# Wells-Group/pmg-dolfinx

Hardware: AMD Instinct MI355X
Metric: DoFs/sec per p-MG V-cycle (Poisson, hex, p=4) (higher is better)
Workload: dtype f64; 1 GPU; Poisson p=4 V-cycle p=4->2->1, Chebyshev(3)/Jacobi, 64^3 hexes per GPU; fine_dofs_global=16974593, partition=1x1x1 bricks, 1 ghost-cell layer, exchange=none (single rank), rccl_ranks=1, comm_ranks=1

## Files before the change

include/pmg_amd.h:

```cpp
#ifndef PMG_AMD_H
#define PMG_AMD_H

#include <stddef.h>
#include <stdint.h>

#ifdef __cplusplus
extern "C" {
#endif

#define PMG_OK 0
#define PMG_ERR_INVALID -1
#define PMG_ERR_HIP -2
#define PMG_ERR_NUMERIC -3
#define PMG_MAX_DEGREE 8

typedef void* pmg_stream;

typedef struct pmg_layout_s* pmg_layout;
typedef struct pmg_comm_s* pmg_comm;
typedef struct pmg_laplacian_s* pmg_laplacian;
typedef struct pmg_chebyshev_s* pmg_chebyshev;
typedef struct pmg_cg_s* pmg_cg;
typedef struct pmg_interpolator_s* pmg_interpolator;
typedef struct pmg_multigrid_s* pmg_multigrid;
// ... 177 lines not shown
                                          const int32_t* bcells, int32_t n_bcells,
                                          pmg_laplacian fine_operator, pmg_stream stream);
int pmg_interpolator_create_ordered(pmg_interpolator* out, pmg_layout layout_coarse, pmg_layout layout_fine,
                                    int degree_coarse, int degree_fine, int32_t ncells,
                                    const int32_t* dofmap_coarse, const int32_t* dofmap_fine,
                                    const int32_t* lcells, int32_t n_lcells, const int32_t* bcells,
                                    int32_t n_bcells, pmg_laplacian fine_operator, int node_order,
                                    const int32_t* custom_coarse, const int32_t* custom_fine, pmg_stream stream);
int pmg_interpolator_destroy(pmg_interpolator ip);
int pmg_interpolator_interpolate(pmg_interpolator ip, double* coarse, double* fine,
                                 pmg_stream stream);
int pmg_interpolator_interpolate_add(pmg_interpolator ip, double* coarse, double* fine,
                                     pmg_stream stream);
int pmg_interpolator_reverse_interpolate(pmg_interpolator ip, double* fine, double* coarse,
                                         pmg_stream stream);
int pmg_interpolator_interpolate_add_f32(pmg_interpolator ip, const float* coarse, float* fine, pmg_stream stream);
int pmg_interpolator_reverse_interpolate_f32(pmg_interpolator ip, const float* fine, const float* fine_sub,
                                             float* coarse, pmg_stream stream);

int pmg_multigrid_create(pmg_multigrid* out, int nlevels, const pmg_layout* layouts,
                         const int8_t* bc_marker_coarsest);
int pmg_multigrid_destroy(pmg_multigrid mg);
int pmg_multigrid_set_operators(pmg_multigrid mg, const pmg_laplacian* ops);
int pmg_multigrid_set_solvers(pmg_multigrid mg, const pmg_chebyshev* smoothers);
int pmg_multigrid_set_interpolators(pmg_multigrid mg, const pmg_interpolator* interp);
int pmg_multigrid_set_coarse_solver(pmg_multigrid mg, pmg_cg coarse);
typedef int (*pmg_coarse_solve_fn)(void* user, double* x, double* b, pmg_stream stream);
int pmg_multigrid_set_coarse_callback(pmg_multigrid mg, pmg_coarse_solve_fn solve, void* user);
int pmg_amg_create(pmg_amg* out, pmg_laplacian op, pmg_stream stream);
int pmg_amg_create_replicated(pmg_amg* out, pmg_laplacian op, const int64_t* global_index, int64_t n_global,
// ... 6 lines not shown
int pmg_amg_set_krylov(pmg_amg amg, int max_iter, double rtol);
int pmg_amg_set_distributed_fine_level(pmg_amg amg, int enable);
int pmg_amg_solve(pmg_amg amg, double* x, const double* b, int* iterations, pmg_stream stream);
int pmg_amg_cycle(pmg_amg amg, double* x, const double* b, pmg_stream stream);
int pmg_amg_num_levels(pmg_amg amg);
int pmg_amg_level_info(pmg_amg amg, int level, long long* rows, long long* nnz, double* lambda_max);
int pmg_amg_export(pmg_amg amg, int level, int which, long long* rows, long long* cols, long long* nnz,
                   int32_t* rowptr, int32_t* colidx, double* values);
int pmg_multigrid_set_coarse_amg(pmg_multigrid mg, pmg_amg amg);

int pmg_multigrid_apply(pmg_multigrid mg, const double* rhs, double* y, double* rnorm,
                        pmg_stream stream);
int pmg_multigrid_set_graph(pmg_multigrid mg, int enable);
long long pmg_multigrid_graph_replays(pmg_multigrid mg);
int pmg_multigrid_apply_counts(pmg_multigrid mg, int* counts, int capacity);
#define PMG_PRECISION_FP64 0
#define PMG_PRECISION_FP32 1
int pmg_multigrid_set_precision(pmg_multigrid mg, int precision);
int pmg_multigrid_set_level_matrix(pmg_multigrid mg, int level, pmg_matrix M);
int pmg_multigrid_precision(pmg_multigrid mg);

#ifdef __cplusplus
}
#endif
#endif
```

pmg-dolfinx_amd/_lib.py:

```python
from __future__ import annotations

import ctypes as C
import os

_HERE = os.path.dirname(os.path.abspath(__file__))
LIB_PATH = os.environ.get("PMG_AMD_LIB") or os.path.join(_HERE, "lib", "libpmg_amd.so")

c_dp = C.POINTER(C.c_double)
c_ip = C.POINTER(C.c_int32)
c_bp = C.POINTER(C.c_int8)
c_lp = C.POINTER(C.c_int64)
vp = C.c_void_p

EXCHANGE_FN = C.CFUNCTYPE(C.c_int, vp, C.c_int, vp)
ALLREDUCE_FN = C.CFUNCTYPE(C.c_int, vp, c_dp, C.c_int)
COARSE_FN = C.CFUNCTYPE(C.c_int, vp, vp, vp, vp)


class PmgError(RuntimeError):
    """A pmg_* call returned non-zero; the message is ``pmg_last_error()``."""


_SIGS = {
    "pmg_last_error": (C.c_char_p, []),
# ... 107 lines not shown
        [C.POINTER(vp), vp, vp, C.c_int, C.c_int, C.c_int32, vp, vp, c_ip, C.c_int32, c_ip, C.c_int32, vp],
    ),
    "pmg_interpolator_create_with_operator": (
        C.c_int,
        [C.POINTER(vp), vp, vp, C.c_int, C.c_int, C.c_int32, vp, vp, c_ip, C.c_int32, c_ip, C.c_int32, vp, vp],
    ),
    "pmg_interpolator_create_ordered": (
        C.c_int,
        [C.POINTER(vp), vp, vp, C.c_int, C.c_int, C.c_int32, vp, vp, c_ip, C.c_int32, c_ip, C.c_int32, vp, C.c_int,
         c_ip, c_ip, vp],
    ),
    "pmg_interpolator_interpolate_add": (C.c_int, [vp, vp, vp, vp]),
    "pmg_interpolator_destroy": (C.c_int, [vp]),
    "pmg_interpolator_interpolate": (C.c_int, [vp, vp, vp, vp]),
    "pmg_interpolator_reverse_interpolate": (C.c_int, [vp, vp, vp, vp]),
    "pmg_interpolator_interpolate_add_f32": (C.c_int, [vp, vp, vp, vp]),
    "pmg_interpolator_reverse_interpolate_f32": (C.c_int, [vp, vp, vp, vp, vp]),
    "pmg_multigrid_create": (C.c_int, [C.POINTER(vp), C.c_int, C.POINTER(vp), vp]),
    "pmg_multigrid_destroy": (C.c_int, [vp]),
    "pmg_multigrid_set_operators": (C.c_int, [vp, C.POINTER(vp)]),
    "pmg_multigrid_set_solvers": (C.c_int, [vp, C.POINTER(vp)]),
    "pmg_multigrid_set_interpolators": (C.c_int, [vp, C.POINTER(vp)]),
    "pmg_multigrid_set_coarse_solver": (C.c_int, [vp, vp]),
    "pmg_multigrid_set_coarse_callback": (C.c_int, [vp, COARSE_FN, vp]),
    "pmg_multigrid_set_coarse_amg": (C.c_int, [vp, vp]),
    "pmg_multigrid_set_precision": (C.c_int, [vp, C.c_int]),
    "pmg_multigrid_precision": (C.c_int, [vp]),
    "pmg_amg_create": (C.c_int, [C.POINTER(vp), vp, vp]),
    "pmg_amg_create_replicated": (C.c_int, [C.POINTER(vp), vp, C.POINTER(C.c_int64), C.c_int64, vp]),
    "pmg_amg_create_distributed": (C.c_int, [C.POINTER(vp), vp, C.POINTER(C.c_int64), C.c_int64, vp]),
# ... 2 lines not shown
    "pmg_amg_set_cycles": (C.c_int, [vp, C.c_int]),
    "pmg_amg_set_krylov": (C.c_int, [vp, C.c_int, C.c_double]),
    "pmg_amg_set_distributed_fine_level": (C.c_int, [vp, C.c_int]),
    "pmg_amg_solve": (C.c_int, [vp, vp, vp, C.POINTER(C.c_int), vp]),
    "pmg_amg_cycle": (C.c_int, [vp, vp, vp, vp]),
    "pmg_amg_num_levels": (C.c_int, [vp]),
    "pmg_amg_level_info": (C.c_int, [vp, C.c_int, C.POINTER(C.c_longlong), C.POINTER(C.c_longlong), c_dp]),
    "pmg_amg_export": (C.c_int, [vp, C.c_int, C.c_int, C.POINTER(C.c_longlong), C.POINTER(C.c_longlong),
                                 C.POINTER(C.c_longlong), c_ip, c_ip, c_dp]),
    "pmg_laplacian_set_geometry_batch": (C.c_int, [vp, C.c_longlong]),
    "pmg_laplacian_geometry_bytes": (C.c_longlong, [vp]),
    "pmg_multigrid_apply": (C.c_int, [vp, vp, vp, c_dp, vp]),
    "pmg_multigrid_apply_counts": (C.c_int, [vp, C.POINTER(C.c_int), C.c_int]),
    "pmg_multigrid_set_graph": (C.c_int, [vp, C.c_int]),
    "pmg_multigrid_graph_replays": (C.c_longlong, [vp]),
    "pmg_matrix_create_from_laplacian": (C.c_int, [C.POINTER(vp), vp, vp]),
    "pmg_matrix_destroy": (C.c_int, [vp]),
    "pmg_matrix_update_values": (C.c_int, [vp, vp]),
    "pmg_matrix_apply": (C.c_int, [vp, vp, vp, vp]),
    "pmg_matrix_get_diag_inverse": (C.c_int, [vp, vp, vp]),
    "pmg_matrix_rows": (C.c_longlong, [vp]),
    "pmg_matrix_nnz": (C.c_longlong, [vp]),
    "pmg_matrix_bytes": (C.c_longlong, [vp]),
    "pmg_matrix_frobenius_norm": (C.c_int, [vp, c_dp]),
    "pmg_matrix_export": (C.c_int, [vp, C.POINTER(C.c_longlong), C.POINTER(C.c_longlong), c_ip, c_ip, c_dp]),
    "pmg_chebyshev_solve_matrix": (C.c_int, [vp, vp, vp, vp, vp]),
    "pmg_cg_solve_matrix": (C.c_int, [vp, vp, vp, vp, vp, C.POINTER(C.c_int), vp]),
    "pmg_multigrid_set_level_matrix": (C.c_int, [vp, C.c_int, vp]),
}

_COUNT_FUNCS = {"pmg_multigrid_graph_replays", "pmg_amg_num_levels", "pmg_laplacian_geometry_bytes", "pmg_comm_rank", "pmg_comm_size", "pmg_comm_capture_overlaps", "pmg_cg_coefficients", "pmg_cg_compute_eigenvalues", "pmg_multigrid_apply_counts", "pmg_version",
                "pmg_laplacian_degree", "pmg_multigrid_precision", "pmg_laplacian_launches_per_apply", "pmg_laplacian_apply_streams", "pmg_laplacian_is_affine",
                "pmg_laplacian_has_coefficient_field", "pmg_laplacian_lift_cell_count",
                "pmg_laplacian_chain_available", "pmg_laplacian_chain_form",
                "pmg_laplacian_node_order", "pmg_layout_forward_scatters",
                "pmg_matrix_rows", "pmg_matrix_nnz", "pmg_matrix_bytes"}

_lib = None


def exported_symbols():
    return sorted(_SIGS)


def lib():
    global _lib
    if _lib is None:
        if not os.path.exists(LIB_PATH):
            raise RuntimeError(
                f"{LIB_PATH} is missing: the HIP library has not been built. "
                "Run `python -c 'import __graft_entry__ as g; g.build()'` at the repo root. "
# ... 44 lines not shown
```

pmg-dolfinx_amd/csrc/common.hpp:

```cpp
#pragma once

#include "../../include/pmg_amd.h"

#include <hip/hip_runtime.h>

#include <cstdarg>
#include <cstdio>
#include <functional>
#include <string>
#include <vector>

namespace pmg
{
extern thread_local std::string g_last_error;

int fail(int code, const char* fmt, ...);

#define PMG_HIP(call)                                                                              \
  do                                                                                               \
  {                                                                                                \
    hipError_t e_ = (call);                                                                        \
    if (e_ != hipSuccess)                                                                          \
      return pmg::fail(PMG_ERR_HIP, "%s failed: %s (%s:%d)", #call, hipGetErrorString(e_),         \
                       __FILE__, __LINE__);                                                        \
// ... 135 lines not shown
  ~Range() { range_pop(); }
};

struct ChebWork
{
  double *r = nullptr, *z = nullptr, *q = nullptr;
};
using ApplyFn = std::function<int(double* in, double* out)>;
using PrecondFn = std::function<int(double* z, const double* r)>;
int cg_iterate(pmg_cg cg, const ApplyFn& A, const double* dinv, const PrecondFn* M, bool flexible, double* x,
               const double* b, int* iterations, hipStream_t s);
enum : int
{
  ResidualNone = 0,
  ResidualUpdated = 1,
  ResidualSplit = 2
};
int cheb_iterate(const ChebWork& w, const ApplyFn& A, const double* dinv, int n, double lmax, int max_iter,
                 double* x, const double* b, int need_r, bool x_zero, hipStream_t s, bool* split = nullptr,
                 const ApplyFn* A_zeroed = nullptr, int n_total = 0, bool track_ghosts = false,
                 const ApplyFn* A_first = nullptr);

int dot_async(pmg_layout l, const double* a, const double* b, int slot, hipStream_t s);
double* red_slot(pmg_layout l, int slot);
int reduce_slots_async(pmg_layout l, int slot, int n, bool max, hipStream_t s);
int fetch_slots(pmg_layout l, int slot, int n, double* host_out, hipStream_t s);
int dot_host(pmg_layout l, const double* a, const double* b, double* result, hipStream_t s);
void launch_axpy(int n, double* r, double alpha, const double* x, const double* y, hipStream_t s);
void launch_pointwise(int n, double* w, const double* x, const double* y, hipStream_t s);
void launch_cheb_init(int n, double* r, double* z, const double* b, const double* q,
                      const double* dinv, double c0, hipStream_t s, double* clear_q = nullptr, int n_total = 0);
// ... 40 lines not shown
```

pmg-dolfinx_amd/csrc/interpolate.hip:

```cpp
#include "common.hpp"
#include "patches.hpp"

#include <algorithm>
#include <cstdlib>
#include <map>

using namespace pmg;

namespace pmg
{
PatchView laplacian_patches(pmg_laplacian op);
pmg_layout laplacian_layout(pmg_laplacian op);
}

struct pmg_interpolator_s
{
  pmg_layout lc = nullptr, lf = nullptr;
  int pc = 0, pf = 0, ndc = 0, ndf = 0, Nc = 0, Nf = 0;
  int32_t ncells = 0;
  const int32_t* dmc = nullptr;
  const int32_t* dmf = nullptr;
  int32_t* dmc_own = nullptr;
  int32_t* dmf_own = nullptr;
  double* M1 = nullptr;
  float* M1_32 = nullptr;
  double* inv_mult = nullptr;
  int32_t* lcells = nullptr;
// ... 625 lines not shown
}

int interp_prolong_add(pmg_interpolator ip, double* coarse, double* fine, hipStream_t s)
{
  PMG_REQUIRE(ip->patched, "interp_prolong_add needs the patch path");
  return prolong_patched(ip, coarse, fine, 1, s);
}

bool interp_restricts_difference(pmg_interpolator ip) { return ip->patched && ip->lf->num_ghosts == 0; }

int interp_restrict_difference(pmg_interpolator ip, double* fine, const double* fine_sub, double* coarse,
                               hipStream_t s)
{
  PMG_REQUIRE(interp_restricts_difference(ip), "interp_restrict_difference: not available for this interpolator");
  return restrict_patched(ip, fine, fine_sub, coarse, s);
}

int interp_prolong(pmg_interpolator ip, double* coarse, double* fine, hipStream_t s)
{
  if (ip->patched)
    return prolong_patched(ip, coarse, fine, 0, s);
  const size_t shm = sizeof(double) * (ip->ndf * ip->ndc + (size_t)ip->cpb * ip->Nc);
  PMG_TRY(pmg_scatter_fwd_begin(ip->lc, coarse, (pmg_stream)s));
  if (ip->n_l > 0)
    prolong_kernel<<<(ip->n_l + ip->cpb - 1) / ip->cpb, ip->threads, shm, s>>>(
        ip->n_l, ip->lcells, ip->cpb, ip->ndc, ip->ndf, ip->dmc, ip->dmf, ip->M1, coarse, fine);
  PMG_TRY(pmg_scatter_fwd_end(ip->lc, coarse, (pmg_stream)s));
  if (ip->n_b > 0)
    prolong_kernel<<<(ip->n_b + ip->cpb - 1) / ip->cpb, ip->threads, shm, s>>>(
        ip->n_b, ip->bcells, ip->cpb, ip->ndc, ip->ndf, ip->dmc, ip->dmf, ip->M1, coarse, fine);
// ... 218 lines not shown
  (*out)->dmc_own = own[0];
  (*out)->dmf_own = own[1];
  return PMG_OK;
}

extern "C" int pmg_interpolator_interpolate_add(pmg_interpolator ip, double* coarse, double* fine,
                                                pmg_stream stream)
{
  PMG_REQUIRE(ip && coarse && fine, "pmg_interpolator_interpolate_add: NULL argument");
  if (ip->patched)
    return interp_prolong_add(ip, coarse, fine, S(stream));
  return fail(PMG_ERR_INVALID, "pmg_interpolator_interpolate_add needs an interpolator created "
                               "with pmg_interpolator_create_with_operator");
}

extern "C" int pmg_interpolator_destroy(pmg_interpolator ip)
{
  if (!ip)
    return PMG_OK;
  (void)hipFree(ip->dmc_own);
  (void)hipFree(ip->dmf_own);
  (void)hipFree(ip->cpoff);
  (void)hipFree(ip->cpdofs);
  (void)hipFree(ip->clmap_id);
  (void)hipFree(ip->clmaps);
  (void)hipFree(ip->pmult);
  (void)hipFree(ip->M1);
  (void)hipFree(ip->M1_32);
  (void)hipFree(ip->inv_mult);
  (void)hipFree(ip->lcells);
// ... 19 lines not shown
```

pmg-dolfinx_amd/csrc/laplacian.hip:

```cpp
#include "laplacian.hpp"

#include <algorithm>
#include <cmath>
#include <cstdlib>
#include <type_traits>

using namespace pmg;


namespace
{
#include "geometry_kernels.hpp"
#include "stiffness_column.hpp"
#include "stiffness_chain.hpp"

__global__ void zero_list_kernel(int n, const int32_t* __restrict__ idx, double* __restrict__ y)
{
  for (int i = blockIdx.x * blockDim.x + threadIdx.x; i < n; i += gridDim.x * blockDim.x)
    y[idx[i]] = 0.0;
}

const double2* batch_geometry(pmg_laplacian op, int first, int count, hipStream_t s)
{
  double2* base = op->G - (size_t)first * gpatch(op->nd, op->K);
  const long long nslots = (long long)count * op->K, n = nslots * op->N;
  if (n > 0)
    geometry_kernel<<<(unsigned)((n + 255) / 256), 256, 0, s>>>((long long)first * op->K, nslots, op->nd, op->K,
                                                              op->pcell, op->xgeom, op->geom_dofmap,
                                                              op->dphi_geom, op->gweights, op->kfield, op->dofmap,
// ... 178 lines not shown
    op->prof_used += 2;
    op->prof_launches += issued;
  }
  return PMG_OK;
}

template <typename T>
int upload(T** dst, const T* src, size_t n, hipStream_t s)
{
  PMG_HIP(hipMalloc(dst, sizeof(T) * (n ? n : 1)));
  if (n)
    PMG_HIP(hipMemcpyAsync(*dst, src, sizeof(T) * n, hipMemcpyHostToDevice, s));
  return PMG_OK;
}

}

namespace pmg
{
int laplacian_apply(pmg_laplacian op, double* in, double* out, hipStream_t s);
int laplacian_apply_zeroed(pmg_laplacian op, double* in, double* out, hipStream_t s);
int laplacian_apply_ghosts_current(pmg_laplacian op, double* in, double* out, hipStream_t s);
const double* laplacian_diag_inv(pmg_laplacian op) { return op->diag_inv; }
pmg_layout laplacian_layout(pmg_laplacian op) { return op->layout; }
long long laplacian_launches(pmg_laplacian op) { return op->applies; }
struct LaplacianInputs
{
  int degree;
  int32_t ncells;
  const int32_t* dofmap;
  const int8_t* bc;
  const double* kappa;
};
LaplacianInputs laplacian_inputs(pmg_laplacian op) { return {op->P, op->ncells, op->dofmap, op->bc, op->kappa}; }
// ... 715 lines not shown
```

pmg-dolfinx_amd/csrc/solvers.hip:

```cpp
#include "common.hpp"

#include <cstdlib>

#include <algorithm>
#include <cmath>
#include <cstring>

using namespace pmg;

namespace pmg
{
int laplacian_apply(pmg_laplacian op, double* in, double* out, hipStream_t s);
const double* laplacian_diag_inv(pmg_laplacian op);
pmg_layout laplacian_layout(pmg_laplacian op);
long long laplacian_launches(pmg_laplacian op);
int interp_prolong(pmg_interpolator ip, double* coarse, double* fine, hipStream_t s);
int interp_restrict(pmg_interpolator ip, double* fine, double* coarse, hipStream_t s);
int interp_prolong_add(pmg_interpolator ip, double* coarse, double* fine, hipStream_t s);
bool interp_is_patched(pmg_interpolator ip);
bool interp_restricts_difference(pmg_interpolator ip);
int interp_restrict_difference(pmg_interpolator ip, double* fine, const double* fine_sub, double* coarse,
                               hipStream_t s);
int amg_solve(pmg_amg amg, double* x, const double* b, hipStream_t s);
pmg_layout amg_layout(pmg_amg amg);
long long amg_capture_state(pmg_amg amg);
long long laplacian_capture_state(pmg_laplacian op);
void launch_cheb_first(int n, double* x, double* r, double* z, const double* q, const double* dinv,
                       double c1, double c2, int x_final, hipStream_t s, double* clear_q = nullptr, int n_total = 0);
bool laplacian_wants_zeroed_output(pmg_laplacian op);
int laplacian_apply_zeroed(pmg_laplacian op, double* in, double* out, hipStream_t s);
int laplacian_apply_ghosts_current(pmg_laplacian op, double* in, double* out, hipStream_t s);
int matrix_apply(pmg_matrix M, const double* in, double* out, hipStream_t s);
const double* matrix_diag_inv(pmg_matrix M);
pmg_layout matrix_layout(pmg_matrix M);
}

struct pmg_chebyshev_s
// ... 28 lines not shown
  std::vector<int> counts;
  pmg_cg coarse = nullptr;
  pmg_coarse_solve_fn coarse_fn = nullptr;
  void* coarse_user = nullptr;
  pmg_amg coarse_amg = nullptr;
  std::vector<pmg_matrix> mats;
  std::vector<long long> mat_applies;
  struct GraphEntry
  {
    const double* rhs;
    double* y;
    bool y_zero;
    uint64_t config;
    hipGraphExec_t exec;
    std::vector<int> counts;
  };
  int graph_mode = -1;
  std::vector<GraphEntry> graphs;
  hipStream_t capture_stream = nullptr;
  long long graph_replays = 0;
  int precision = PMG_PRECISION_FP64;
  std::vector<float*> u32, b32;
  std::vector<ChebWork32> w32;
  std::vector<const float*> dinv32;
  std::vector<const float*> M1_32;
};

namespace pmg
{
int cheb_iterate(const ChebWork& w, const ApplyFn& A, const double* dinv, int n, double lmax, int max_iter,
                 double* x, const double* b, int need_r, bool x_zero, hipStream_t s, bool* split,
                 const ApplyFn* A_zeroed, int n_total, bool track_ghosts, const ApplyFn* A_first)
{
  if (split)
    *split = false;
// ... 12 lines not shown
    PMG_TRY(A_first ? (*A_first)(x, w.q) : A(x, w.q));
    launch_cheb_init(n, w.r, w.z, b, w.q, dinv, c0, s, clear_q, n_total);
  }
  for (int i = 1; i <= max_iter; ++i)
  {
    const bool last = (i == max_iter);
    if (last && !need_r)
    {
      if (max_iter == 1)
      {
        if (x_zero)
          PMG_HIP(hipMemcpyAsync(x, w.z, sizeof(double) * n, hipMemcpyDeviceToDevice, s));
        else
          launch_add(n, x, w.z, s);
      }
      break;
    }
    PMG_TRY(An(w.z, w.q));
    if (ng > 0)
      launch_add(ng, x + n, w.z + n, s);
    if (last)
    {
      if (max_iter == 1)
        launch_cheb_last(n, x, w.r, w.z, w.q, x_zero, s);
      else if (need_r == ResidualSplit && split)
        *split = true;
      else
        launch_cheb_residual(n, w.r, w.q, s);
      break;
    }
// ... 46 lines not shown
                      hipStream_t s, bool* split = nullptr, long long* applies = nullptr)
{
  pmg_layout l = sm->layout;
  PMG_REQUIRE(matrix_layout(M) == l, "Chebyshev: matrix and smoother layouts differ");
  const ChebWork w{sm->r, sm->z, sm->q};
  const ApplyFn apply = [M, s, applies](double* in, double* out)
  {
    if (applies)
      ++*applies;
    return matrix_apply(M, in, out, s);
  };
  return cheb_iterate(w, apply, matrix_diag_inv(M), l->size_local, sm->eig_max, sm->max_iter, x, b, need_r, x_zero, s,
                      split);
}

int level_smooth(pmg_multigrid mg, int i, double* x, const double* b, int need_r, bool x_zero, hipStream_t s,
                 bool* split = nullptr, bool track_ghosts = false, bool x_ghosts_current = false)
{
  if (mg->mats[i])
    return cheb_solve_matrix(mg->smoothers[i], mg->mats[i], x, b, need_r, x_zero, s, split, &mg->mat_applies[i]);
  return cheb_solve(mg->smoothers[i], mg->ops[i], x, b, need_r, x_zero, s, split, track_ghosts, x_ghosts_current);
}

long long level_applies(pmg_multigrid mg, int i) { return laplacian_launches(mg->ops[i]) + mg->mat_applies[i]; }

bool local_correction(pmg_multigrid mg, int level)
{
  if (const char* e = std::getenv("PMG_LOCAL_CORRECTION"))
    if (e[0] == '0')
      return false;
// ... 64 lines not shown
  mg->M1_32.assign(L - 1, nullptr);
  for (int i = 0; i < L - 1; ++i)
    PMG_TRY(transfer_f32_prepare(mg->interps[i], &mg->M1_32[i]));
  mg->dinv32.assign(L, nullptr);
  for (int i = 0; i < L; ++i)
  {
    PMG_TRY(laplacian_f32_prepare(mg->ops[i], s));
    PMG_TRY(laplacian_f32_diag(mg->ops[i], &mg->dinv32[i], s, nullptr));
  }
  return PMG_OK;
}

int mg_apply_f32(pmg_multigrid mg, const double* rhs, double* y, bool y_zero, hipStream_t s)
{
  const int L = mg->L;
  std::vector<long long> before(L);
  for (int i = 0; i < L; ++i)
    before[i] = laplacian_launches(mg->ops[i]);
  PMG_TRY(mg_prepare_f32(mg, s));
  Range cycle("pmg:vcycle_f32");
  const int nf = mg->layouts[L - 1]->size_local;
  if (y_zero)
    launch_to_f32(nf, rhs, nullptr, mg->b32[L - 1], s);
  else
  {
    double* q = mg->smoothers[L - 1]->q;
    PMG_TRY(laplacian_apply(mg->ops[L - 1], y, q, s));
    launch_to_f32(nf, rhs, q, mg->b32[L - 1], s);
  }
  for (int i = L - 1; i > 0; --i)
// ... 62 lines not shown
}

int mg_apply(pmg_multigrid mg, const double* rhs, double* y, bool y_zero, hipStream_t s)
{
  const int L = mg->L;
  PMG_REQUIRE((int)mg->ops.size() == L && (int)mg->smoothers.size() == L
                  && (int)mg->interps.size() == L - 1,
              "MultigridPreconditioner: operators / solvers / interpolators not set");
  if (mg->precision == PMG_PRECISION_FP32)
    return mg_apply_f32(mg, rhs, y, y_zero, s);
  std::vector<long long> before(L);
  for (int i = 0; i < L; ++i)
    before[i] = level_applies(mg, i);
  Range cycle("pmg:vcycle");
  mg->u[L - 1] = y;
  for (int i = L - 1; i > 0; --i)
  {
    const double* bi = (i == L - 1) ? rhs : mg->b[i];
    const bool zero = (i == L - 1) ? y_zero : true;
    bool split = false;
    {
      Range rg("pmg:pre_smooth");
      PMG_TRY(level_smooth(mg, i, mg->u[i], bi,
                           interp_restricts_difference(mg->interps[i - 1]) ? ResidualSplit : ResidualUpdated, zero, s,
                           &split, local_correction(mg, i)));
    }
    Range rg("pmg:restrict");
    if (split)
      PMG_TRY(interp_restrict_difference(mg->interps[i - 1], mg->smoothers[i]->r, mg->smoothers[i]->q,
                                         mg->b[i - 1], s));
    else
      PMG_TRY(interp_restrict(mg->interps[i - 1], mg->smoothers[i]->r, mg->b[i - 1], s));
  }
  if (L > 1)
    launch_mask_bc(mg->layouts[0]->size_local, mg->b[0], mg->bc0, s);
  {
    Range rg("pmg:coarse_solve");
    const double* b0 = (L == 1) ? rhs : mg->b[0];
    const bool zero = (L == 1) ? y_zero : true;
    if (mg->coarse_amg && L > 1)
      PMG_TRY(amg_solve(mg->coarse_amg, mg->u[0], mg->b[0], s));
    else if ((mg->coarse || mg->coarse_fn) && L > 1)
    {
// ... 478 lines not shown
    mix((uint64_t)(uintptr_t)mg->smoothers[i]);
    mix((uint64_t)(uintptr_t)mg->mats[i]);
    mix((uint64_t)(uintptr_t)l->comm);
    mix((uint64_t)(uintptr_t)l->win);
    if (i + 1 < mg->L)
      mix((uint64_t)(uintptr_t)mg->interps[i]);
    mix((uint64_t)mg->smoothers[i]->max_iter);
    uint64_t bits;
    static_assert(sizeof(bits) == sizeof(double), "");
    memcpy(&bits, &mg->smoothers[i]->eig_max, sizeof(bits));
    mix(bits);
  }
  if (mg->coarse || mg->coarse_fn)
    return -1;
  mix((uint64_t)mg->precision);
  if (mg->precision == PMG_PRECISION_FP32)
    for (int i = 0; i < mg->L; ++i)
      mix((uint64_t)laplacian_diag_version(mg->ops[i]));
  if (mg->coarse_amg)
  {
    const long long st = amg_capture_state(mg->coarse_amg);
    if (st < 0)
      return -1;
    mix((uint64_t)st);
    mix((uint64_t)(uintptr_t)mg->coarse_amg);
  }
  return (long long)(h >> 1);
}

int mg_apply_graph(pmg_multigrid mg, const double* rhs, double* y, bool y_zero, hipStream_t s, bool* done)
{
  *done = false;
  if ((int)mg->ops.size() != mg->L || (int)mg->smoothers.size() != mg->L || (int)mg->interps.size() != mg->L - 1)
    return PMG_OK;
  const long long cfg = capture_config(mg);
  if (cfg < 0)
    return PMG_OK;
  for (auto& g : mg->graphs)
    if (g.rhs == rhs && g.y == y && g.y_zero == y_zero && g.config == (uint64_t)cfg)
    {
      PMG_HIP(hipGraphLaunch(g.exec, s));
      mg->counts = g.counts;
      mg->graph_replays++;
      *done = true;
      return PMG_OK;
    }
  if (mg->precision == PMG_PRECISION_FP32)
    PMG_TRY(mg_prepare_f32(mg, s));
  if (!mg->capture_stream)
    PMG_HIP(hipStreamCreateWithFlags(&mg->capture_stream, hipStreamNonBlocking));
  PMG_HIP(hipStreamBeginCapture(mg->capture_stream, hipStreamCaptureModeRelaxed));
  const int rc = mg_apply(mg, rhs, y, y_zero, mg->capture_stream);
  hipGraph_t graph = nullptr;
  const hipError_t e = hipStreamEndCapture(mg->capture_stream, &graph);
  if (rc != PMG_OK)
  {
    if (graph)
      (void)hipGraphDestroy(graph);
    return rc;
  }
  if (e != hipSuccess || !graph)
    return fail(PMG_ERR_HIP, "capturing the V-cycle failed: %s", hipGetErrorString(e));
  pmg_multigrid_s::GraphEntry g{rhs, y, y_zero, (uint64_t)cfg, nullptr, mg->counts};
  const hipError_t ei = hipGraphInstantiate(&g.exec, graph, nullptr, nullptr, 0);
  (void)hipGraphDestroy(graph);
  if (ei != hipSuccess)
    return fail(PMG_ERR_HIP, "instantiating the V-cycle graph failed: %s", hipGetErrorString(ei));
  if (mg->graphs.size() >= 16)
    drop_graphs(mg);
  mg->graphs.push_back(g);
  PMG_HIP(hipGraphLaunch(g.exec, s));
  mg->graph_replays++;
  *done = true;
  return PMG_OK;
}
}

extern "C" int pmg_multigrid_set_graph(pmg_multigrid mg, int enable)
{
  PMG_REQUIRE(mg, "pmg_multigrid_set_graph: NULL argument");
  drop_graphs(mg);
  mg->graph_mode = enable < 0 ? -1 : (enable != 0 ? 1 : 0);
  return PMG_OK;
}

extern "C" int pmg_multigrid_set_precision(pmg_multigrid mg, int precision)
{
  PMG_REQUIRE(mg, "pmg_multigrid_set_precision: NULL argument");
  PMG_REQUIRE(precision == PMG_PRECISION_FP64 || precision == PMG_PRECISION_FP32,
              "pmg_multigrid_set_precision: unknown precision %d (PMG_PRECISION_FP64 or PMG_PRECISION_FP32)", precision);
  if (precision == PMG_PRECISION_FP32)
  {
    for (int i = 0; i < mg->L; ++i)
      PMG_REQUIRE(!mg->mats[i],
                  "pmg_multigrid_set_precision: level %d has an assembled matrix and there is no FP32 matrix "
                  "(pmg_multigrid_set_level_matrix(mg, %d, NULL) removes it)", i, i);
    PMG_TRY(mg_check_f32(mg, "pmg_multigrid_set_precision"));
  }
  drop_graphs(mg);
  mg->precision = precision;
// ... 58 lines not shown
```

pmg-dolfinx_amd/interpolate.py:

```python
from __future__ import annotations

import ctypes as C

import numpy as np

from . import _lib
from ._lib import call, current_stream, ptr, vp
from .laplacian import _dev_i32, node_order_args
from .vector import Layout, Vector


class Interpolator:

    def __init__(self, Q1_degree, Q2_degree, Q1_dofmap, Q2_dofmap, l_cells, b_cells, Q1_layout: Layout,
                 Q2_layout: Layout, fine_operator=None, node_order="ascending", perm1d_coarse=None,
                 perm1d_fine=None):
        dev = Q2_layout.device
        self.lc, self.lf = Q1_layout, Q2_layout
        self.dmc = _dev_i32(Q1_dofmap, dev)
        self.dmf = _dev_i32(Q2_dofmap, dev)
        Nc, Nf = (Q1_degree + 1) ** 3, (Q2_degree + 1) ** 3
        ncells = int(self.dmf.numel() // Nf)
        if self.dmc.numel() // Nc != ncells:
            raise ValueError("coarse and fine dofmaps describe different numbers of cells")
# ... 15 lines not shown
    def handle(self):
        return self._handle

    def interpolate(self, Q1_vector: Vector, Q2_vector: Vector):
        call("pmg_interpolator_interpolate", self._handle, ptr(Q1_vector.data), ptr(Q2_vector.data),
             current_stream())

    def interpolate_add(self, Q1_vector: Vector, Q2_vector: Vector):
        call("pmg_interpolator_interpolate_add", self._handle, ptr(Q1_vector.data), ptr(Q2_vector.data),
             current_stream())

    def reverse_interpolate(self, Q2_vector: Vector, Q1_vector: Vector):
        call("pmg_interpolator_reverse_interpolate", self._handle, ptr(Q2_vector.data), ptr(Q1_vector.data),
             current_stream())

    def interpolate_add_fp32(self, coarse, fine):
        self._check_fp32(coarse=(coarse, self.lc), fine=(fine, self.lf))
        call("pmg_interpolator_interpolate_add_f32", self._handle, vp(coarse.data_ptr()), vp(fine.data_ptr()),
             current_stream())

    def reverse_interpolate_fp32(self, fine, coarse, fine_sub=None):
        vecs = dict(fine=(fine, self.lf), coarse=(coarse, self.lc))
        if fine_sub is not None:
            vecs["fine_sub"] = (fine_sub, self.lf)
        self._check_fp32(**vecs)
        call("pmg_interpolator_reverse_interpolate_f32", self._handle, vp(fine.data_ptr()),
             vp(fine_sub.data_ptr()) if fine_sub is not None else vp(0), vp(coarse.data_ptr()), current_stream())

    @staticmethod
    def _check_fp32(**vecs):
# ... 17 lines not shown
```

pmg-dolfinx_amd/pmg.py:

```python
from __future__ import annotations

import ctypes as C

from . import _lib
from ._lib import call, current_stream, ptr, vp
from .laplacian import _dev_i8
from .vector import Vector


class MultigridPreconditioner:

    def __init__(self, layouts, bc_marker_coarsest, bs: int = 1):
        self.layouts = list(layouts)
        self.bc0 = _dev_i8(bc_marker_coarsest, self.layouts[0].device)
        arr = (vp * len(self.layouts))(*[l.handle for l in self.layouts])
        h = vp()
        call("pmg_multigrid_create", C.byref(h), len(self.layouts), arr, ptr(self.bc0))
        self._handle = h
        self._keep = {}

    @property
    def handle(self):
        return self._handle

# ... 55 lines not shown
            call("pmg_multigrid_set_coarse_callback", self._handle, self._keep["coarse_cb"], None)
        else:
            raise TypeError("the coarse solver needs a solve(x, b) method")

    def apply(self, x: Vector, y: Vector, verbose: bool = False):
        if verbose:
            rn = C.c_double()
            call("pmg_multigrid_apply", self._handle, ptr(x.data), ptr(y.data), C.byref(rn), current_stream())
            return rn.value
        call("pmg_multigrid_apply", self._handle, ptr(x.data), ptr(y.data), None, current_stream())
        return None

    def set_graph(self, enable=True):
        call("pmg_multigrid_set_graph", self._handle, -1 if enable is None else (1 if enable else 0))

    PRECISIONS = {"fp64": 0, "fp32": 1}

    def set_precision(self, precision: str):
        if precision not in self.PRECISIONS:
            raise ValueError(f"precision must be one of {sorted(self.PRECISIONS)}, not {precision!r}")
        call("pmg_multigrid_set_precision", self._handle, self.PRECISIONS[precision])

    @property
    def precision(self) -> str:
        code = call("pmg_multigrid_precision", self._handle)
        return {v: k for k, v in self.PRECISIONS.items()}[code]

    def graph_replays(self) -> int:
        return call("pmg_multigrid_graph_replays", self._handle)

# ... 14 lines not shown
```

Baseline: 3.471 billion DoF/s.

## Fuse final smoother operator apply, residual and restriction into one kernel

Adds a stiffness_restrict kernel that applies the fine-level operator to the last Chebyshev update, forms the residual per patch in shared memory, and restricts it straight into the coarse right-hand side with LDS and global atomics. The pre-smoother stops before its last operator apply (ResidualFused) and the V-cycle calls this fused restriction when the interpolator and operator share patches and the degree pair is 2-1, 4-2, 3-1 or 6-3. It is on by default. The goal is to skip writing and re-reading the fine residual vector and one kernel launch per level, at the cost of a heavier kernel with more shared memory and atomics.

```diff
diff --git a/include/pmg_amd.h b/include/pmg_amd.h
--- a/include/pmg_amd.h
+++ b/include/pmg_amd.h
@@ -215,6 +215,8 @@
                                      pmg_stream stream);
 int pmg_interpolator_reverse_interpolate(pmg_interpolator ip, double* fine, double* coarse,
                                          pmg_stream stream);
+int pmg_interpolator_restrict_residual(pmg_interpolator ip, pmg_laplacian op, const double* z, const double* r,
+                                       double* coarse, pmg_stream stream);
 int pmg_interpolator_interpolate_add_f32(pmg_interpolator ip, const float* coarse, float* fine, pmg_stream stream);
 int pmg_interpolator_reverse_interpolate_f32(pmg_interpolator ip, const float* fine, const float* fine_sub,
                                              float* coarse, pmg_stream stream);
@@ -251,6 +253,8 @@
 int pmg_multigrid_set_graph(pmg_multigrid mg, int enable);
 long long pmg_multigrid_graph_replays(pmg_multigrid mg);
 int pmg_multigrid_apply_counts(pmg_multigrid mg, int* counts, int capacity);
+int pmg_multigrid_set_fused_restriction(pmg_multigrid mg, int mode);
+int pmg_multigrid_fused_restrictions(pmg_multigrid mg);
 #define PMG_PRECISION_FP64 0
 #define PMG_PRECISION_FP32 1
 int pmg_multigrid_set_precision(pmg_multigrid mg, int precision);
diff --git a/pmg-dolfinx_amd/_lib.py b/pmg-dolfinx_amd/_lib.py
--- a/pmg-dolfinx_amd/_lib.py
+++ b/pmg-dolfinx_amd/_lib.py
@@ -145,6 +145,7 @@
     "pmg_interpolator_destroy": (C.c_int, [vp]),
     "pmg_interpolator_interpolate": (C.c_int, [vp, vp, vp, vp]),
     "pmg_interpolator_reverse_interpolate": (C.c_int, [vp, vp, vp, vp]),
+    "pmg_interpolator_restrict_residual": (C.c_int, [vp, vp, vp, vp, vp, vp]),
     "pmg_interpolator_interpolate_add_f32": (C.c_int, [vp, vp, vp, vp]),
     "pmg_interpolator_reverse_interpolate_f32": (C.c_int, [vp, vp, vp, vp, vp]),
     "pmg_multigrid_create": (C.c_int, [C.POINTER(vp), C.c_int, C.POINTER(vp), vp]),
@@ -177,6 +178,8 @@
     "pmg_multigrid_apply_counts": (C.c_int, [vp, C.POINTER(C.c_int), C.c_int]),
     "pmg_multigrid_set_graph": (C.c_int, [vp, C.c_int]),
     "pmg_multigrid_graph_replays": (C.c_longlong, [vp]),
+    "pmg_multigrid_set_fused_restriction": (C.c_int, [vp, C.c_int]),
+    "pmg_multigrid_fused_restrictions": (C.c_int, [vp]),
     "pmg_matrix_create_from_laplacian": (C.c_int, [C.POINTER(vp), vp, vp]),
     "pmg_matrix_destroy": (C.c_int, [vp]),
     "pmg_matrix_update_values": (C.c_int, [vp, vp]),
@@ -197,7 +200,7 @@
                 "pmg_laplacian_has_coefficient_field", "pmg_laplacian_lift_cell_count",
                 "pmg_laplacian_chain_available", "pmg_laplacian_chain_form",
                 "pmg_laplacian_node_order", "pmg_layout_forward_scatters",
-                "pmg_matrix_rows", "pmg_matrix_nnz", "pmg_matrix_bytes"}
+                "pmg_matrix_rows", "pmg_matrix_nnz", "pmg_matrix_bytes", "pmg_multigrid_fused_restrictions"}
 
 _lib = None
 
diff --git a/pmg-dolfinx_amd/csrc/common.hpp b/pmg-dolfinx_amd/csrc/common.hpp
--- a/pmg-dolfinx_amd/csrc/common.hpp
+++ b/pmg-dolfinx_amd/csrc/common.hpp
@@ -173,7 +173,8 @@
 {
   ResidualNone = 0,
   ResidualUpdated = 1,
-  ResidualSplit = 2
+  ResidualSplit = 2,
+  ResidualFused = 3
 };
 int cheb_iterate(const ChebWork& w, const ApplyFn& A, const double* dinv, int n, double lmax, int max_iter,
                  double* x, const double* b, int need_r, bool x_zero, hipStream_t s, bool* split = nullptr,
diff --git a/pmg-dolfinx_amd/csrc/interpolate.hip b/pmg-dolfinx_amd/csrc/interpolate.hip
--- a/pmg-dolfinx_amd/csrc/interpolate.hip
+++ b/pmg-dolfinx_amd/csrc/interpolate.hip
@@ -11,6 +11,9 @@
 {
 PatchView laplacian_patches(pmg_laplacian op);
 pmg_layout laplacian_layout(pmg_laplacian op);
+bool laplacian_fuses_restriction(pmg_laplacian op, int coarse_degree);
+int laplacian_apply_restrict(pmg_laplacian op, const TransferView& tv, const double* z, const double* r,
+                             double* coarse, hipStream_t s);
 }
 
 struct pmg_interpolator_s
@@ -666,6 +669,22 @@
 {
   PMG_REQUIRE(interp_restricts_difference(ip), "interp_restrict_difference: not available for this interpolator");
   return restrict_patched(ip, fine, fine_sub, coarse, s);
+}
+
+bool interp_fuses_residual(pmg_interpolator ip, pmg_laplacian op)
+{
+  return ip->patched && op && ip->lf->num_ghosts == 0 && laplacian_layout(op) == ip->lf
+         && laplacian_patches(op).pdofs == ip->fv.pdofs && laplacian_fuses_restriction(op, ip->pc);
+}
+
+int interp_restrict_residual(pmg_interpolator ip, pmg_laplacian op, const double* z, const double* r, double* coarse,
+                             hipStream_t s)
+{
+  PMG_REQUIRE(interp_fuses_residual(ip, op),
+              "the fused residual restriction is not available here: it needs a patch-form interpolator on the patches "
+              "of this operator, fine vectors without ghosts, resident geometry and one of the degree pairs 1-2, 2-4, "
+              "1-3, 3-6");
+  return laplacian_apply_restrict(op, interp_transfer_view(ip), z, r, coarse, s);
 }
 
 int interp_prolong(pmg_interpolator ip, double* coarse, double* fine, hipStream_t s)
@@ -914,6 +933,13 @@
                                "with pmg_interpolator_create_with_operator");
 }
 
+extern "C" int pmg_interpolator_restrict_residual(pmg_interpolator ip, pmg_laplacian op, const double* z,
+                                                  const double* r, double* coarse, pmg_stream stream)
+{
+  PMG_REQUIRE(ip && op && z && r && coarse, "pmg_interpolator_restrict_residual: NULL argument");
+  return interp_restrict_residual(ip, op, z, r, coarse, S(stream));
+}
+
 extern "C" int pmg_interpolator_destroy(pmg_interpolator ip)
 {
   if (!ip)
diff --git a/pmg-dolfinx_amd/csrc/laplacian.hip b/pmg-dolfinx_amd/csrc/laplacian.hip
--- a/pmg-dolfinx_amd/csrc/laplacian.hip
+++ b/pmg-dolfinx_amd/csrc/laplacian.hip
@@ -13,6 +13,7 @@
 #include "geometry_kernels.hpp"
 #include "stiffness_column.hpp"
 #include "stiffness_chain.hpp"
+#include "stiffness_restrict.hpp"
 
 __global__ void zero_list_kernel(int n, const int32_t* __restrict__ idx, double* __restrict__ y)
 {
@@ -221,10 +222,67 @@
   return PMG_OK;
 }
 
+#define PMG_FOR_FUSED_PAIRS(X) X(2, 1) X(4, 2) X(3, 1) X(6, 3)
+
+template <int P, int PC>
+int launch_stiffness_restrict(pmg_laplacian op, const TransferView& tv, const double* z, const double* r,
+                              double* coarse, hipStream_t s)
+{
+  constexpr int cm = RestrictShape<P, PC>::CM;
+  PMG_REQUIRE(tv.cmax_m <= cm, "internal: a patch holds %d coarse dofs, the fused kernel %d", tv.cmax_m, cm);
+  const RestrictLists R{tv.cpoff, tv.clmap_id, tv.cpdofs, tv.clmaps, tv.pmult, tv.M1};
+  const bool nt = P >= NT_FROM && op->geometry_mode != 1 && op->stream_policy;
+#define PMG_LAUNCH_FUSED(AFF_, NT_)                                                                                  \
+  stiffness_restrict_kernel<P, PC, AFF_, NT_><<<op->npatch, Shape<P>::WTHREADS, 0, s>>>(                             \
+      z, r, coarse, op->G, op->Gaff, op->W1, op->poff, op->pdofs, op->lmap_id, op->lmaps, op->pcell, op->pncell,     \
+      op->kappa, op->D, R)
+  if (op->geometry_mode == 1)
+    PMG_LAUNCH_FUSED(true, false);
+  else if (nt)
+    PMG_LAUNCH_FUSED(false, true);
+  else
+    PMG_LAUNCH_FUSED(false, false);
+#undef PMG_LAUNCH_FUSED
+  PMG_HIP(hipGetLastError());
+  return PMG_OK;
+}
+
 }
 
 namespace pmg
 {
+bool laplacian_fuses_restriction(pmg_laplacian op, int coarse_degree)
+{
+  if (op->layout->num_ghosts != 0 || op->batch_patches != 0)
+    return false;
+#define X(F, C)                                                                                                      \
+  if (op->P == F && coarse_degree == C)                                                                              \
+    return true;
+  PMG_FOR_FUSED_PAIRS(X)
+#undef X
+  return false;
+}
+
+int laplacian_apply_restrict(pmg_laplacian op, const TransferView& tv, const double* z, const double* r,
+                             double* coarse, hipStream_t s)
+{
+  PMG_REQUIRE(laplacian_fuses_restriction(op, tv.ndc - 1) && tv.ndf == op->nd && tv.fv.pdofs == op->pdofs
+                  && tv.fv.npatch == op->npatch && tv.lf == op->layout,
+              "laplacian_apply_restrict: not available for this operator and transfer");
+  launch_zero(tv.lc->total(), coarse, s);
+  if (op->npatch > 0)
+  {
+#define X(F, C)                                                                                                      \
+  if (op->P == F && tv.ndc - 1 == C)                                                                                 \
+    PMG_TRY((launch_stiffness_restrict<F, C>(op, tv, z, r, coarse, s)));
+    PMG_FOR_FUSED_PAIRS(X)
+#undef X
+    op->launches++;
+  }
+  op->applies++;
+  return PMG_OK;
+}
+
 int laplacian_apply(pmg_laplacian op, double* in, double* out, hipStream_t s);
 int laplacian_apply_zeroed(pmg_laplacian op, double* in, double* out, hipStream_t s);
 int laplacian_apply_ghosts_current(pmg_laplacian op, double* in, double* out, hipStream_t s);
diff --git a/pmg-dolfinx_amd/csrc/solvers.hip b/pmg-dolfinx_amd/csrc/solvers.hip
--- a/pmg-dolfinx_amd/csrc/solvers.hip
+++ b/pmg-dolfinx_amd/csrc/solvers.hip
@@ -21,6 +21,9 @@
 bool interp_restricts_difference(pmg_interpolator ip);
 int interp_restrict_difference(pmg_interpolator ip, double* fine, const double* fine_sub, double* coarse,
                                hipStream_t s);
+bool interp_fuses_residual(pmg_interpolator ip, pmg_laplacian op);
+int interp_restrict_residual(pmg_interpolator ip, pmg_laplacian op, const double* z, const double* r, double* coarse,
+                             hipStream_t s);
 int amg_solve(pmg_amg amg, double* x, const double* b, hipStream_t s);
 pmg_layout amg_layout(pmg_amg amg);
 long long amg_capture_state(pmg_amg amg);
@@ -79,11 +82,14 @@
     uint64_t config;
     hipGraphExec_t exec;
     std::vector<int> counts;
+    int fused_count;
   };
   int graph_mode = -1;
   std::vector<GraphEntry> graphs;
   hipStream_t capture_stream = nullptr;
   long long graph_replays = 0;
+  int fused_mode = -1;
+  int fused_count = 0;
   int precision = PMG_PRECISION_FP64;
   std::vector<float*> u32, b32;
   std::vector<ChebWork32> w32;
@@ -126,6 +132,11 @@
         else
           launch_add(n, x, w.z, s);
       }
+      break;
+    }
+    if (last && need_r == ResidualFused && split && max_iter > 1)
+    {
+      *split = true;
       break;
     }
     PMG_TRY(An(w.z, w.q));
@@ -202,6 +213,21 @@
                       split);
 }
 
+bool fuses_restriction(pmg_multigrid mg, int i)
+{
+  if (mg->fused_mode == 0 || i <= 0 || mg->mats[i] || !interp_fuses_residual(mg->interps[i - 1], mg->ops[i]))
+    return false;
+  if (const char* e = std::getenv("PMG_FUSED_DEGREES"))
+  {
+    const int P = pmg_laplacian_degree(mg->ops[i]);
+    for (const char* c = e; *c; ++c)
+      if (*c - '0' == P)
+        return true;
+    return false;
+  }
+  return true;
+}
+
 int level_smooth(pmg_multigrid mg, int i, double* x, const double* b, int need_r, bool x_zero, hipStream_t s,
                  bool* split = nullptr, bool track_ghosts = false, bool x_ghosts_current = false)
 {
@@ -296,6 +322,7 @@
 int mg_apply_f32(pmg_multigrid mg, const double* rhs, double* y, bool y_zero, hipStream_t s)
 {
   const int L = mg->L;
+  mg->fused_count = 0;
   std::vector<long long> before(L);
   for (int i = 0; i < L; ++i)
     before[i] = laplacian_launches(mg->ops[i]);
@@ -388,19 +415,29 @@
     before[i] = level_applies(mg, i);
   Range cycle("pmg:vcycle");
   mg->u[L - 1] = y;
+  mg->fused_count = 0;
   for (int i = L - 1; i > 0; --i)
   {
     const double* bi = (i == L - 1) ? rhs : mg->b[i];
     const bool zero = (i == L - 1) ? y_zero : true;
+    const bool fuse = fuses_restriction(mg, i);
     bool split = false;
     {
       Range rg("pmg:pre_smooth");
       PMG_TRY(level_smooth(mg, i, mg->u[i], bi,
-                           interp_restricts_difference(mg->interps[i - 1]) ? ResidualSplit : ResidualUpdated, zero, s,
-                           &split, local_correction(mg, i)));
+                           fuse                                              ? ResidualFused
+                           : interp_restricts_difference(mg->interps[i - 1]) ? ResidualSplit
+                                                                             : ResidualUpdated,
+                           zero, s, &split, local_correction(mg, i)));
     }
     Range rg("pmg:restrict");
-    if (split)
+    if (split && fuse)
+    {
+      PMG_TRY(interp_restrict_residual(mg->interps[i - 1], mg->ops[i], mg->smoothers[i]->z, mg->smoothers[i]->r,
+                                       mg->b[i - 1], s));
+      mg->fused_count++;
+    }
+    else if (split)
       PMG_TRY(interp_restrict_difference(mg->interps[i - 1], mg->smoothers[i]->r, mg->smoothers[i]->q,
                                          mg->b[i - 1], s));
     else
@@ -909,6 +946,7 @@
   if (mg->coarse || mg->coarse_fn)
     return -1;
   mix((uint64_t)mg->precision);
+  mix((uint64_t)(mg->fused_mode + 1));
   if (mg->precision == PMG_PRECISION_FP32)
     for (int i = 0; i < mg->L; ++i)
       mix((uint64_t)laplacian_diag_version(mg->ops[i]));
@@ -936,6 +974,7 @@
     {
       PMG_HIP(hipGraphLaunch(g.exec, s));
       mg->counts = g.counts;
+      mg->fused_count = g.fused_count;
       mg->graph_replays++;
       *done = true;
       return PMG_OK;
@@ -956,7 +995,7 @@
   }
   if (e != hipSuccess || !graph)
     return fail(PMG_ERR_HIP, "capturing the V-cycle failed: %s", hipGetErrorString(e));
-  pmg_multigrid_s::GraphEntry g{rhs, y, y_zero, (uint64_t)cfg, nullptr, mg->counts};
+  pmg_multigrid_s::GraphEntry g{rhs, y, y_zero, (uint64_t)cfg, nullptr, mg->counts, mg->fused_count};
   const hipError_t ei = hipGraphInstantiate(&g.exec, graph, nullptr, nullptr, 0);
   (void)hipGraphDestroy(graph);
   if (ei != hipSuccess)
@@ -979,6 +1018,17 @@
   return PMG_OK;
 }
 
+extern "C" int pmg_multigrid_set_fused_restriction(pmg_multigrid mg, int mode)
+{
+  PMG_REQUIRE(mg, "pmg_multigrid_set_fused_restriction: NULL argument");
+  PMG_REQUIRE(mode == -1 || mode == 0, "pmg_multigrid_set_fused_restriction: mode %d (-1 automatic, 0 never)", mode);
+  drop_graphs(mg);
+  mg->fused_mode = mode;
+  return PMG_OK;
+}
+
+extern "C" int pmg_multigrid_fused_restrictions(pmg_multigrid mg) { return mg ? mg->fused_count : -1; }
+
 extern "C" int pmg_multigrid_set_precision(pmg_multigrid mg, int precision)
 {
   PMG_REQUIRE(mg, "pmg_multigrid_set_precision: NULL argument");
diff --git a/pmg-dolfinx_amd/csrc/stiffness_restrict.hpp b/pmg-dolfinx_amd/csrc/stiffness_restrict.hpp
--- /dev/null
+++ b/pmg-dolfinx_amd/csrc/stiffness_restrict.hpp
@@ -0,0 +1,343 @@
+template <int P, int PC>
+struct RestrictShape
+{
+  using Sh = Shape<P>;
+  static_assert(Sh::WPC == 1 && !transposes_by_identity(P), "the fused form covers the one-wave-per-item shapes only");
+  static constexpr int NDC = PC + 1, NC = NDC * NDC * NDC;
+  static constexpr int CM = Sh::K * NC < Sh::MAXM ? Sh::K * NC : Sh::MAXM;
+  static constexpr int CITER = (CM + Sh::WTHREADS - 1) / Sh::WTHREADS;
+  static constexpr int BCW = Sh::WITER * Sh::WTHREADS / 64;
+};
+
+struct RestrictLists
+{
+  const int32_t *cpoff, *clmap_id;
+  const uint32_t* cpdofs;
+  const uint16_t* clmaps;
+  const uint8_t* pmult;
+  const double* M1;
+};
+
+template <int P>
+constexpr int restrict_waves_per_simd()
+{
+  return P == 2 ? 2 : P == 3 ? 4 : min_waves_per_simd<P>();
+}
+
+template <int P, int PC, bool AFF, bool NT>
+__global__ void __launch_bounds__(Shape<P>::WTHREADS, restrict_waves_per_simd<P>())
+    stiffness_restrict_kernel(const double* __restrict__ z, const double* __restrict__ r, double* __restrict__ coarse,
+                              const double2* __restrict__ G, const double* __restrict__ Gaff,
+                              const double* __restrict__ W1, const int32_t* __restrict__ poff,
+                              const uint32_t* __restrict__ pdofs, const int32_t* __restrict__ lmap_id,
+                              const uint16_t* __restrict__ lmaps, const int32_t* __restrict__ pcell,
+                              const int32_t* __restrict__ pncell, const double* __restrict__ kappa,
+                              const double* __restrict__ Dg, RestrictLists R)
+{
+  using Sh = Shape<P>;
+  using Rs = RestrictShape<P, PC>;
+  constexpr int ND = Sh::ND, N = Sh::N, K = Sh::K, NQ2 = Sh::NQ2, CW = Sh::CW, NG = Sh::NG;
+  constexpr int MAXM = Sh::MAXM, THREADS = Sh::WTHREADS, ITER = Sh::WITER;
+  constexpr int NDC = Rs::NDC, NC = Rs::NC, CM = Rs::CM, CITER = Rs::CITER;
+  constexpr int WL = CW * NQ2;
+  constexpr bool UNPAIRED = unpaired_slice_reads(P);
+  __shared__ double sD[ND * ND];
+  __shared__ double sM[ND * NDC];
+  __shared__ double sW[AFF ? ND : 1];
+  __shared__ double skap[K];
+  __shared__ double sx[MAXM];
+  __shared__ double sy[MAXM];
+  __shared__ double sc[CM];
+  __shared__ unsigned long long sbc[Rs::BCW];
+  __shared__ double ssl[3 * NG * WL];
+  constexpr bool FLAT = !AFF && gflat(ND);
+  constexpr int FL = 3 * WL, NJ = (FL + 63) / 64, LS = gls(ND);
+  __shared__ double2 sgb[FLAT ? NG * NJ * 64 : 1];
+
+  const int p = blockIdx.x;
+  const int t = threadIdx.x;
+  const int off = poff[p];
+  const int M = poff[p + 1] - off;
+  const int table = lmap_id[p];
+  const int nc = pncell[p];
+  const int ctable = __builtin_amdgcn_readfirstlane(R.clmap_id[p]);
+  const int coff = R.cpoff[p];
+  const int Mc = R.cpoff[p + 1] - coff;
+
+  {
+    uint32_t m[ITER];
+    uint8_t mu[ITER];
+#pragma unroll
+    for (int k = 0; k < ITER; ++k)
+    {
+      const int i = t + k * THREADS;
+      const int ic = off + (i < M ? i : M - 1);
+      m[k] = pdofs[ic];
+      mu[k] = R.pmult[ic];
+    }
+    const int cellk = pcell[(size_t)p * K + (t < K ? t : K - 1)];
+    const double dval = Dg[t < ND * ND ? t : ND * ND - 1];
+    const double mval = R.M1[t < ND * NDC ? t : ND * NDC - 1];
+    double zv[ITER], rv[ITER];
+#pragma unroll
+    for (int k = 0; k < ITER; ++k)
+    {
+      const uint32_t dof = m[k] & PD_MASK;
+      zv[k] = z[dof];
+      rv[k] = r[dof];
+    }
+    const double kapk = kappa[cellk >= 0 ? cellk : 0];
+#pragma unroll
+    for (int k = 0; k < ITER; ++k)
+    {
+      const int i = t + k * THREADS;
+      const bool bc = i < M && (m[k] & PD_BC);
+      if (i < M)
+      {
+        sx[i] = bc ? 0.0 : zv[k];
+        sy[i] = (bc ? rv[k] - zv[k] : rv[k]) / (double)mu[k];
+      }
+      const unsigned long long rows = __builtin_amdgcn_ballot_w64(bc);
+      if ((t & 63) == 0)
+        sbc[i >> 6] = rows;
+    }
+    if (t < ND * ND)
+      sD[t] = dval;
+    if (t < ND * NDC)
+      sM[t] = mval;
+    if constexpr (AFF)
+    {
+      if (t < ND)
+        sW[t] = W1[t];
+    }
+    for (int i = t; i < K; i += THREADS)
+      skap[i] = (i == t) ? kapk : kappa[pcell[(size_t)p * K + i] >= 0 ? pcell[(size_t)p * K + i] : 0];
+    for (int i = t; i < CM; i += THREADS)
+      sc[i] = 0.0;
+  }
+  lds_barrier();
+
+  const int wave = t >> 6, lane = t & 63;
+  const bool lane_ok = lane < WL;
+  const int lw = lane_ok ? lane : WL - 1;
+  const int cw = lw / NQ2;
+  const int ab = lw - cw * NQ2;
+  const int a = ab / ND, b = ab - a * ND;
+  double Da[ND], Db[ND], DTa[ND], DTb[ND];
+#pragma unroll
+  for (int mm = 0; mm < ND; ++mm)
+  {
+    Da[mm] = sD[a * ND + mm];
+    Db[mm] = sD[b * ND + mm];
+    DTa[mm] = sD[mm * ND + a];
+    DTb[mm] = sD[mm * ND + b];
+  }
+  double* q_s = ssl + wave * WL + cw * NQ2;
+  double* gr_s = q_s + NG * WL;
+  double* gs_s = q_s + 2 * NG * WL;
+  const bool coarse_ok = lane_ok && a < NDC && b < NDC;
+  auto coarse_point = [](int abv, int& i, int& j, int bound) {
+    asm volatile("" : "+v"(abv));
+    const int av = abv / ND, bv = abv - av * ND;
+    i = av < bound ? av : bound - 1;
+    j = bv < bound ? bv : bound - 1;
+  };
+  const int items = (nc + CW - 1) / CW;
+
+  for (int it = wave; it < items; it += NG)
+  {
+    const int slot = it * CW + cw;
+    const int slotc = slot < K ? slot : K - 1;
+    const uint16_t* lmb = lmaps + (size_t)table * (K * N);
+    const unsigned lmo = (unsigned)(slotc * N + ab);
+    constexpr int GPS = NQ2;
+    const double2* Gb = G + (size_t)p * ((long long)K * 3 * N);
+    const unsigned Gs = (unsigned)(slotc * 3 * N + ab);
+    int l[ND];
+#pragma unroll
+    for (int k = 0; k < ND; ++k)
+      l[k] = lmb[lmo + (unsigned)(k * NQ2)];
+    const uint16_t* clb = R.clmaps + (size_t)ctable * (K * NC);
+    int ic, jc;
+    coarse_point(ab, ic, jc, NDC);
+    const unsigned clo = (unsigned)(slotc * NC + (ic * NDC + jc) * NDC);
+    unsigned lcp[(NDC + 1) / 2];
+#pragma unroll
+    for (int k = 0; k < NDC; k += 2)
+      lcp[k / 2] = (unsigned)clb[clo + (unsigned)k] | (k + 1 < NDC ? (unsigned)clb[clo + (unsigned)(k + 1)] << 16 : 0u);
+#pragma unroll
+    for (int j = 0; j < (NDC + 1) / 2; ++j)
+      asm volatile("" : "+v"(lcp[j]));
+    double2 gq[3];
+    double2 gfl[FLAT ? NJ : 1];
+    const double2* Gi = G + (size_t)p * gpatch(ND, K) + (size_t)__builtin_amdgcn_readfirstlane(it) * ND * LS;
+    int eo[FLAT ? NJ : 1];
+    if constexpr (FLAT)
+    {
+#pragma unroll
+      for (int jj = 0; jj < NJ; ++jj)
+        eo[jj] = lane + 64 * jj < FL ? lane + 64 * jj : FL - 1;
+    }
+    double gc[6] = {0, 0, 0, 0, 0, 0};
+    if constexpr (AFF)
+    {
+      const double* ga = Gaff + ((size_t)p * K + slotc) * 6;
+      int av, bv;
+      coarse_point(ab, av, bv, ND);
+      const double wab = skap[slotc] * (sW[av] * sW[bv]);
+#pragma unroll
+      for (int d = 0; d < 6; ++d)
+        gc[d] = wab * ga[d];
+    }
+    else if constexpr (FLAT)
+    {
+#pragma unroll
+      for (int jj = 0; jj < NJ; ++jj)
+        gfl[jj] = gload<NT>(Gi + eo[jj]);
+    }
+    else
+    {
+      gq[0] = gload<NT>(Gb + Gs);
+      gq[1] = gload<NT>(Gb + (Gs + (unsigned)GPS));
+      gq[2] = gload<NT>(Gb + (Gs + (unsigned)(2 * GPS)));
+    }
+    const double kap = AFF ? 1.0 : skap[slotc];
+    double u[ND], Aq[ND];
+#pragma unroll
+    for (int k = 0; k < ND; ++k)
+    {
+      u[k] = sx[l[k]];
+      Aq[k] = 0.0;
+    }
+    unsigned lp[(ND + 1) / 2];
+#pragma unroll
+    for (int k = 0; k < ND; k += 2)
+      lp[k / 2] = (unsigned)l[k] | (k + 1 < ND ? (unsigned)l[k + 1] << 16 : 0u);
+#pragma unroll
+    for (int j = 0; j < (ND + 1) / 2; ++j)
+      asm volatile("" : "+v"(lp[j]));
+#pragma unroll
+    for (int k = 0; k < ND; ++k)
+    {
+      double2 g01, g23, g45;
+      if constexpr (AFF)
+      {
+        g01 = make_double2(gc[0], gc[1]);
+        g23 = make_double2(gc[2], gc[3]);
+        g45 = make_double2(gc[4], gc[5]);
+      }
+      else if constexpr (FLAT)
+      {
+        double2* gb = sgb + wave * (NJ * 64);
+#pragma unroll
+        for (int jj = 0; jj < NJ; ++jj)
+          gb[lane + 64 * jj] = gfl[jj];
+        wave_fence();
+        g01 = gb[lw];
+        g23 = gb[WL + lw];
+        g45 = gb[2 * WL + lw];
+        if (k + 1 < ND)
+        {
+#pragma unroll
+          for (int jj = 0; jj < NJ; ++jj)
+            gfl[jj] = gload<NT>(Gi + (k + 1) * LS + eo[jj]);
+        }
+      }
+      else
+      {
+        g01 = gq[0];
+        g23 = gq[1];
+        g45 = gq[2];
+        if (k + 1 < ND)
+        {
+          gq[0] = gload<NT>(Gb + (Gs + (unsigned)((k + 1) * 3 * GPS)));
+          gq[1] = gload<NT>(Gb + (Gs + (unsigned)((k + 1) * 3 * GPS + GPS)));
+          gq[2] = gload<NT>(Gb + (Gs + (unsigned)((k + 1) * 3 * GPS + 2 * GPS)));
+        }
+      }
+      q_s[ab] = u[k];
+      wave_fence();
+      double qr = 0.0, qs = 0.0, qt = 0.0;
+#pragma unroll
+      for (int mm = 0; mm < ND; ++mm)
+      {
+        qr += Da[mm] * slice_load<UNPAIRED>(q_s[mm * ND + b]);
+        qs += Db[mm] * slice_load<UNPAIRED>(q_s[a * ND + mm]);
+        qt += Dg[k * ND + mm] * u[mm];
+      }
+      const double sck = AFF ? W1[k] : kap;
+      const double fr = sck * (g01.x * qr + g01.y * qs + g23.x * qt);
+      const double fs = sck * (g01.y * qr + g23.y * qs + g45.x * qt);
+      const double ft = sck * (g23.x * qr + g45.x * qs + g45.y * qt);
+      double acc = 0.0;
+      gr_s[ab] = fr;
+      gs_s[ab] = fs;
+      wave_fence();
+#pragma unroll
+      for (int mm = 0; mm < ND; ++mm)
+      {
+        acc += DTa[mm] * slice_load<UNPAIRED>(gr_s[mm * ND + b]);
+        acc += DTb[mm] * slice_load<UNPAIRED>(gs_s[a * ND + mm]);
+        Aq[mm] += Dg[k * ND + mm] * ft;
+      }
+      Aq[k] += acc;
+      wave_fence();
+    }
+    int ie, je;
+    coarse_point(ab, ie, je, NDC);
+    double w[ND];
+#pragma unroll
+    for (int k = 0; k < ND; ++k)
+    {
+      const int lk = (int)((lp[k / 2] >> (16 * (k & 1))) & 0xffffu);
+      const bool bc = (sbc[lk >> 6] >> (lk & 63)) & 1ull;
+      w[k] = sy[lk] - (bc ? 0.0 : Aq[k]);
+    }
+    double tz[NDC];
+#pragma unroll
+    for (int k = 0; k < NDC; ++k)
+    {
+      tz[k] = 0.0;
+#pragma unroll
+      for (int c = 0; c < ND; ++c)
+        tz[k] += R.M1[c * NDC + k] * w[c];
+    }
+    const bool contributes = coarse_ok && slot < nc;
+#pragma unroll
+    for (int k = 0; k < NDC; ++k)
+    {
+      q_s[ab] = tz[k];
+      wave_fence();
+      double vx = 0.0;
+#pragma unroll
+      for (int mm = 0; mm < ND; ++mm)
+        vx += sM[mm * NDC + ie] * q_s[mm * ND + b];
+      gr_s[ab] = vx;
+      wave_fence();
+      double vy = 0.0;
+#pragma unroll
+      for (int mm = 0; mm < ND; ++mm)
+        vy += sM[mm * NDC + je] * gr_s[ie * ND + mm];
+      if (contributes)
+        atomicAdd(&sc[(lcp[k / 2] >> (16 * (k & 1))) & 0xffffu], vy);
+      wave_fence();
+    }
+  }
+  int tw = t;
+  asm volatile("" : "+v"(tw));
+  uint32_t cm[CITER];
+#pragma unroll
+  for (int j = 0; j < CITER; ++j)
+  {
+    const int i = tw + j * THREADS;
+    cm[j] = R.cpdofs[coff + (i < Mc ? i : Mc - 1)];
+  }
+  lds_barrier();
+#pragma unroll
+  for (int j = 0; j < CITER; ++j)
+  {
+    const int i = tw + j * THREADS;
+    if (i < Mc)
+      atomicAdd(&coarse[cm[j] & PD_MASK], sc[i]);
+  }
+}
diff --git a/pmg-dolfinx_amd/interpolate.py b/pmg-dolfinx_amd/interpolate.py
--- a/pmg-dolfinx_amd/interpolate.py
+++ b/pmg-dolfinx_amd/interpolate.py
@@ -53,6 +53,10 @@
         call("pmg_interpolator_reverse_interpolate", self._handle, ptr(Q2_vector.data), ptr(Q1_vector.data),
              current_stream())
 
+    def restrict_residual(self, operator, z: Vector, r: Vector, Q1_vector: Vector):
+        call("pmg_interpolator_restrict_residual", self._handle, operator.handle, ptr(z.data), ptr(r.data),
+             ptr(Q1_vector.data), current_stream())
+
     def interpolate_add_fp32(self, coarse, fine):
         self._check_fp32(coarse=(coarse, self.lc), fine=(fine, self.lf))
         call("pmg_interpolator_interpolate_add_f32", self._handle, vp(coarse.data_ptr()), vp(fine.data_ptr()),
diff --git a/pmg-dolfinx_amd/pmg.py b/pmg-dolfinx_amd/pmg.py
--- a/pmg-dolfinx_amd/pmg.py
+++ b/pmg-dolfinx_amd/pmg.py
@@ -93,6 +93,13 @@
     def set_graph(self, enable=True):
         call("pmg_multigrid_set_graph", self._handle, -1 if enable is None else (1 if enable else 0))
 
+    def set_fused_restriction(self, mode=None):
+        code = -1 if mode is None or mode is True else int(mode)
+        call("pmg_multigrid_set_fused_restriction", self._handle, code)
+
+    def fused_restrictions(self) -> int:
+        return call("pmg_multigrid_fused_restrictions", self._handle)
+
     PRECISIONS = {"fp64": 0, "fp32": 1}
 
     def set_precision(self, precision: str):
```

Result: faster. 3.602 billion DoF/s, median of 6 (+3.8%).
